# Hevagog/as-cops-and-thieves

Measured on AMD Instinct MI355X. Metric: env-steps/sec (whole node) at 4096 parallel envs, 2v1 agents, 64-ray sensors, higher is better.
Workload: dtype f64; 1 GPU; 2 cops vs 1 thieves, labyrinth map (30 hull walls / 119 planes), 4096 envs per GPU, 64 rays/agent, dt=1/60, max_step_count=400, Philox random actions, auto-reset; envs_per_gpu=4096, rays=64, agents=3, map=labyrinth, parallelism=env-sharded x1, no data-path collective, episodes_reset_per_gpu=32768, burn_in_steps=600

## Files before the change

as_cops_and_thieves_amd/csrc/cat_sim_fan.h:

```cpp
constexpr int kFeatNear = 63;
constexpr int kItemCap = 128;
constexpr int kPassJ = 8;
constexpr int kFanBytes = 2 * kItemCap * 8 + kItemCap * 2 + kPassJ * kLanes * 2;
constexpr int kGroupRays = 256;

__device__ __forceinline__ void poly_query_feat(const Lds &L, float cmax, bool wall, int sh, double r, double cx, double cy, double ax, double ay,
                                                double bx, double by, double r2, double &alpha, int &feat)
{
    const int fc = wall ? L.fc[sh] : 0, first = fc & 0xFFFF, count = fc >> 16;
    const double rsum = r + r2, rr = rsum * rsum;
    const float axf = (float)ax, ayf = (float)ay;
    const float dxf = (float)(bx - ax), dyf = (float)(by - ay);
    const float len2 = dxf * dxf + dyf * dyf, len = sqrtf(len2);
    const float e1 = 1e-6f * (fabsf(axf) + fabsf(ayf) + cmax + 512.0f);
    const float thr = ((float)rsum + 0.01f) * len * 1.00001f + 0.25f + 64.0f * e1;
    const float s_lo = -((float)rsum + 1.0f) * len, s_hi = len2 + ((float)rsum + 1.0f) * len;
    const bool bevels = rsum > 0.0;
    unsigned pm = 0u, vm = wall ? 0u : 1u;
    const double *pl0 = L.planes + 8 * first;
    {
        typedef float f32x2 __attribute__((ext_vector_type(2)));
        const float *q = L.p32 + kPairF * (wall ? L.fp[sh] : 0);
        const f32x2 ax2 = {axf, axf}, ay2 = {ayf, ayf}, dx2 = {dxf, dxf}, dy2 = {dyf, dyf};
        const f32x2 len3 = {3.0f * len, 3.0f * len}, four = {4.0f, 4.0f};
// ... 815 lines not shown
                    L.itm[t] = (unsigned short)(lane | (id << 6) | ((i - i0) << 12));
                    L.itbb[t] = tbb;
                }
                L.itemidx[(jj - jj0) * kLanes + lane] = (unsigned short)t;
                n_items += c;
            }
            const int jj1 = jj;
            wave_sync();
            PHASE(pc, 5);
            for (int t0 = 0; t0 < n_items; t0 += kLanes) {
                const int t = t0 + lane;
                if (t < n_items) {
                    const int d = L.itm[t];
                    const int il = d & 63, id = (d >> 6) & 63, ia = i0 + (d >> 12);
                    const int g2 = L.alist[r0 + il];
                    const int k2 = ((g2 >> 6) - (ia - i0) * cpa) * kLanes + (g2 & 63);
                    const double2 o2 = *reinterpret_cast<const double2 *>(L.fpos + 2 * ia);
                    const double cbx = o2.x + L.rayd[2 * k2], cby = o2.y + L.rayd[2 * k2 + 1];
                    double alpha = 2.0;
                    int feat = 0;
                    {
                        const bool wall = id < S;
                        const int j = wall ? 0 : id - S;
                        const bool inside = wall ? (id == L.anear[2 * ia] || id == L.anear[2 * ia + 1]) : ((((unsigned)L.adn[ia] >> j) & 1u) != 0u);
                        if (inside) { alpha = 0.0; feat = kFeatNear; }
                        else {
                            int f;
                            poly_query_feat(L, cmax, wall, wall ? id : 0, wall ? wall_r : rc, L.ftc[2 * j], L.ftc[2 * j + 1], o2.x, o2.y, cbx, cby, r2, alpha, f);
                            feat = f < 0 ? 0 : f;
                        }
                    }
                    L.ialpha[t] = alpha; L.itm[t] = (unsigned short)((id << 6) | feat);
                }
            }
            wave_sync();
            PHASE(pc, 6);
            for (int q = jj0; q < jj1; q++) {
                const int t = cnt > q ? (int)L.itemidx[(q - jj0) * kLanes + lane] : 0xFFFF;
                if (t != 0xFFFF) {
                    const double al = L.ialpha[t];
                    if (al < best_a && L.itbb[t] < best_a) { best_a = al; best_fi = L.itm[t]; }
                }
            }
            wave_sync();
            PHASE(pc, 7);
            jj0 = jj1;
        }
        unsigned d16 = d_empty, ty = CAT_EMPTY;
        int best = -1;
        if (best_fi >= 0) {
            const double bx = ax + L.rayd[2 * k], by = ay + L.rayd[2 * k + 1];
            best = best_fi >> 6;
            const int f = best_fi & 63;
            const double t = best_a;
            double px = bx, py = by;
            if (f != kFeatNear) {
                const bool wall = best < S;
                const int fc = wall ? L.fc[best] : 0, first = fc & 0xFFFF, count = fc >> 16;
                if (wall && f < count) {
                    const double2 n = *reinterpret_cast<const double2 *>(L.planes + 8 * (first + f));
                    px = (ax * (1.0 - t) + bx * t) - n.x * r2;
                    py = (ay * (1.0 - t) + by * t) - n.y * r2;
                } else {
                    double2 v = *reinterpret_cast<const double2 *>(L.planes + 8 * (first + (wall ? f - count : 0)) + 2);
                    if (!wall) { v.x = L.ftc[2 * (best - S)]; v.y = L.ftc[2 * (best - S) + 1]; }
                    circle_hit_point(v.x, v.y, ax, ay, bx, by, t, r2, px, py);
                }
            }
            d16 = obs_distance_f16(px, py, ax, ay);
            ty = (best < S) ? CAT_WALL : ((best - S) >= n_cops ? CAT_THIEF : CAT_COP);
        }
        if (on) {
            const int q = i * R + k;
            L.od[q] = (unsigned short)d16;
            L.ot[q] = (unsigned char)ty;
            if (la.out.hit_shape) la.out.hit_shape[(size_t)env * A * R + q] = best;
            const unsigned want = i < n_cops ? CAT_THIEF : CAT_COP;
            if (rew_mode && ty == want) __hip_atomic_fetch_min(&L.dmin[i], d16, __ATOMIC_RELAXED, __HIP_MEMORY_SCOPE_WORKGROUP);
        }
        PHASE(pc, 8);
    }
}

template <class D>
__device__ void rewards_and_positions(const Lds &L, const Params &p, const LaunchArgs &la, int lane, int rew_mode,
                                      int captured, int timeout, GAS const float *cop_lut, GAS const float *thief_lut, LateOut &late)
{
    const int A = D::A(p);
    late.reward = 0.0f; late.tp16 = 0;
    if (rew_mode && lane < A && la.out.reward) {
        const unsigned my_dmin = L.dmin[lane];
        const bool is_cop = lane < D::n_cops(p);
        float r;
        if (captured) r = is_cop ? 1.0f : -1.0f;
        else if (timeout) r = is_cop ? -1.0f : 1.0f;
        else if (my_dmin < 0x10000u) r = (is_cop ? cop_lut : thief_lut)[my_dmin & 0x7FFFu];
        else r = is_cop ? (float)(-0.02 - 0.02) : (float)0.15;
        late.reward = r;
    }
    if (lane < 2 * A) late.tp16 = f64_to_f16(L.fpos[lane]);
}
__device__ __forceinline__ void await_reward(LateOut &late) { asm volatile("" : "+v"(late.reward)); }

__device__ __forceinline__ void wide_store(void *gdst, const void *lsrc, int n, int lane)
{
    const unsigned long long ga = (unsigned long long)gdst;
    if (((ga | (unsigned)n) & 15u) == 0) {
        for (int o = lane; o < n / 16; o += kLanes) ((GAS u32x4 *)gdst)[o] = reinterpret_cast<const u32x4 *>(lsrc)[o];
    } else if (((ga | (unsigned)n) & 3u) == 0) {
        for (int o = lane; o < n / 4; o += kLanes) ((GAS unsigned *)gdst)[o] = reinterpret_cast<const unsigned *>(lsrc)[o];
    } else if (((ga | (unsigned)n) & 1u) == 0) {
        for (int o = lane; o < n / 2; o += kLanes) ((GAS unsigned short *)gdst)[o] = reinterpret_cast<const unsigned short *>(lsrc)[o];
    } else {
        for (int o = lane; o < n; o += kLanes) ((GAS unsigned char *)gdst)[o] = reinterpret_cast<const unsigned char *>(lsrc)[o];
    }
}

template <class D>
__device__ __forceinline__ void stage_shared_observations(const Lds &L, const Params &p, int lane)
{
    const int A = D::A(p), R = D::R(p);
    for (int k = lane; k < R; k += kLanes) {
        for (int team = 0; team < 2; team++) {
            const int lo = team ? D::n_cops(p) : 0, hi = team ? A : D::n_cops(p);
            unsigned ty = CAT_EMPTY, d = 0;
            for (int i = lo; i < hi; i++)
                if (ty == CAT_EMPTY) { ty = L.ot[i * R + k]; d = L.od[i * R + k]; }
            L.st[team * R + k] = (unsigned char)ty;
            L.sd[team * R + k] = (unsigned short)d;
        }
    }
    wave_sync();
}

template <class D>
__device__ __forceinline__ void emit_observations(const Lds &L, const Params &p, const LaunchArgs &la, long long env, int lane,
                                                  int rew_mode, const LateOut &late)
{
    const int A = D::A(p), R = D::R(p);
    if (rew_mode && lane < A && la.out.reward) la.out.reward[(size_t)env * A + lane] = late.reward;
    if (lane < 2 * A && la.out.team_positions) la.out.team_positions[(size_t)env * A * 2 + lane] = (unsigned short)late.tp16;
    const size_t g0 = (size_t)env * A * R;
    if (la.out.obs_distance) wide_store(la.out.obs_distance + g0, L.od, A * R * 2, lane);
    if (la.out.obs_type) wide_store(la.out.obs_type + g0, L.ot, A * R, lane);
    if (la.out.shared_distance) wide_store(la.out.shared_distance + (size_t)env * 2 * R, L.sd, 2 * R * 2, lane);
    if (la.out.shared_type) wide_store(la.out.shared_type + (size_t)env * 2 * R, L.st, 2 * R, lane);
}

template <class D>
__device__ int termination_captured(const Lds &L, const Params &p, int S, int lane)
{
    const int A = D::A(p), nc = D::n_cops(p), npairs = (A - nc) * nc;
    bool within = false;
    if (lane < npairs) {
        const int t = nc + lane / nc, c = lane % nc;
        const double ddx = L.pos[2 * t] - L.pos[2 * c], ddy = L.pos[2 * t + 1] - L.pos[2 * c + 1];
        within = sqrt(ddx * ddx + ddy * ddy) < p.term_radius;
    }
    unsigned long long cand = __ballot(within);
    while (cand) {
        {
            const int pair = __builtin_ctzll(cand);
            cand &= cand - 1;
            const int t = nc + pair / nc, c = pair % nc;
            const double ax = L.pos[2 * t], ay = L.pos[2 * t + 1], bx = L.pos[2 * c], by = L.pos[2 * c + 1];
            const double dx = bx - ax, dy = by - ay, idx = 1.0 / dx, idy = 1.0 / dy;
            bool any = false;
            for (int base = 0; base < S; base += kLanes) {
                const int s = base + lane;
                bool hit = false;
                if (s < S) {
                    bool visit = true;
                    if (p.gate && !(D::kTree && S == 1)) visit = bb_segment_query(L.bb + kBB * s, ax, ay, dx, dy, idx, idy) < 1.0;
                    if (visit) {
                        SegInfo info = {0, 1.0, bx, by};
                        if (poly_point_distance(L, s, p.wall_r, ax, ay) <= 0.0) { info.hit = 1; info.alpha = 0.0; }
                        else poly_segment_query(L, s, p.wall_r, ax, ay, bx, by, 0.0, info);
                        hit = info.hit && info.alpha < 1.0;
                    }
                }
                any = any || (__ballot(hit) != 0ull);
            }
            if (!any) return 1;
// ... 5 lines not shown
```

as_cops_and_thieves_amd/csrc/cat_sim_scheduler.h:

```cpp
template <class D>
__device__ __forceinline__ Lds carve(const Params &p, char *smem, const MapDesc &md, int slot, int wave)
{
    Lds L;
    const int S = md.S, P = md.P, W = p.wpb;
    L.bb = reinterpret_cast<const double *>(smem);
    L.planes = L.bb + kBB * S;
    L.p32 = reinterpret_cast<const float *>(L.planes + 8 * P);
    L.fc = reinterpret_cast<const int *>(L.planes + geo_rest_doubles(md));
    L.fp = L.fc + S;
    L.rayd = reinterpret_cast<const double *>(smem + p.lds_map_bytes - 16 * D::R(p));
    L.ctrl = reinterpret_cast<int *>(smem + p.lds_map_bytes);
    char *w = smem + p.lds_map_bytes + ctrl_bytes(W) + slot * p.lds_env_bytes;
    const int A = D::A(p), R = D::R(p), NPs = D::NP(p) > 0 ? D::NP(p) : 1;
    L.rec = w;
    double *d = reinterpret_cast<double *>(w);
    L.pos = d; d += 2 * A; L.vel = d; d += 2 * A; L.vb = d; d += 2 * A; L.tc = d; d += 2 * A;
    L.leaf = d; d += 4 * A;
    L.cnt = reinterpret_cast<int *>(d);
    d = reinterpret_cast<double *>(w + D::hot_bytes(p));
    L.wjn = d; d += A * kK; L.pjn = d; d += NPs;
    {
        int *ri = reinterpret_cast<int *>(d);
        L.wsh = ri; ri += A * kK; L.wag = ri; ri += A * kK; L.pag = ri;
    }
// ... 67 lines not shown
        dm.S = m.S; dm.P = m.P; dm.A = m.A; dm.n_regions = m.n_regions; dm.f64_off = m.f64_off; dm.i32_off = m.i32_off; dm.cmax = m.cmax; dm.PP = m.PP;
        dg.x0 = g.x0; dg.y0 = g.y0; dg.inv_cell = g.inv_cell; dg.nx = g.nx; dg.ny = g.ny; dg.off_base = g.off_base; dg.ent_base = g.ent_base;
        dg.coff_base = g.coff_base; dg.cent_base = g.cent_base; dg.crow_base = g.crow_base; dg.span = g.span; dg.row_base = g.row_base; dg.span_tick = g.span_tick;
    }
    __syncthreads();
}

template <class D>
__device__ __forceinline__ void load_cold(const Lds &L, const Params &p, int env, int lane)
{
    const int A = D::A(p), NPs = D::NP(p) > 0 ? D::NP(p) : 1;
    const int hot16 = D::hot_bytes(p) / 16, cold16 = (D::rec_bytes(p) - D::hot_bytes(p)) / 16;
    u32x4 *dst = reinterpret_cast<u32x4 *>(L.rec) + hot16;
    if (uni(L.cnt[3]) != 0) {
        GAS const u32x4 *src = (GAS const u32x4 *)(G(p.state) + (size_t)env * D::rec_bytes(p)) + hot16;
        for (int o = lane; o < cold16; o += kLanes) dst[o] = src[o];
    } else {
        const int nd2 = 2 * (A * kK + NPs);
        for (int o = lane; o < cold16; o += kLanes) {
            u32x4 v;
#pragma unroll
            for (int q = 0; q < 4; q++) {
                const int j = 4 * o + q - nd2;
                v[q] = (j >= 0 && (j < A * kK || (j >= 2 * A * kK && j < 2 * A * kK + NPs))) ? 0xFFFFFFFFu : 0u;
            }
            dst[o] = v;
        }
    }
    wave_sync();
}

template <class D>
__device__ __forceinline__ void load_state(const Lds &L, const Params &p, int env, int lane)
{
    GAS const u32x4 *src = (GAS const u32x4 *)(G(p.state) + (size_t)env * D::rec_bytes(p));
    u32x4 *dst = reinterpret_cast<u32x4 *>(L.rec);
    for (int o = lane; o < D::hot_bytes(p) / 16; o += kLanes) dst[o] = src[o];
    wave_sync();
    load_cold<D>(L, p, env, lane);
}

struct StateRegs { u32x4 v; };
template <class D>
__device__ __forceinline__ void fetch_state(StateRegs &r, const Params &p, int env, int lane)
{
    GAS const u32x4 *src = (GAS const u32x4 *)(G(p.state) + (size_t)(env < 0 ? 0 : env) * D::rec_bytes(p));
    if (lane < D::hot_bytes(p) / 16) r.v = src[lane];
}
template <class D>
__device__ __forceinline__ void commit_state(const Lds &L, const StateRegs &r, const Params &p, int lane)
{
    u32x4 *dst = reinterpret_cast<u32x4 *>(L.rec);
    if (lane < D::hot_bytes(p) / 16) dst[lane] = r.v;
    wave_sync();
}

template <class D>
__device__ __forceinline__ void store_state(const Lds &L, const Params &p, int env, int lane)
{
    wave_sync();
    const int A = D::A(p);
    const bool mine = (lane < A * kK && L.wsh[lane] >= 0) || (lane < D::NP(p) && L.pag[lane] >= 0);
    const bool live = __ballot(mine) != 0ull;
    if (lane == 0) L.cnt[3] = live ? 1 : 0;
    wave_sync();
    GAS u32x4 *dst = (GAS u32x4 *)(G(p.state) + (size_t)env * D::rec_bytes(p));
    const u32x4 *src = reinterpret_cast<const u32x4 *>(L.rec);
    const int n16 = (live ? D::rec_bytes(p) : D::hot_bytes(p)) / 16;
    for (int o = lane; o < n16; o += kLanes) dst[o] = src[o];
}

#ifdef CAT_WAVE_SPREAD
__device__ unsigned long long g_wave_t[8 * 65536];
__device__ unsigned long long g_slot_t[16 * 65536];
extern "C" int cat_debug_spread(unsigned long long *out, int n)
{
    return hipMemcpyFromSymbol(out, HIP_SYMBOL(g_wave_t), sizeof(unsigned long long) * 8 * n) == hipSuccess ? 0 : -1;
}
extern "C" int cat_debug_slot_times(unsigned long long *out, int n)
{
    return hipMemcpyFromSymbol(out, HIP_SYMBOL(g_slot_t), sizeof(unsigned long long) * 16 * n) == hipSuccess ? 0 : -1;
}
#define SSPREAD(slot_, i) do { if (kOneTick && lane0 == 0 && (i) < 14) g_slot_t[16 * (blockIdx.x * (blockDim.x / kLanes) + (slot_)) + (i)] = __builtin_amdgcn_s_memrealtime(); } while (0)
#define WSPREAD(i) do { if (kOneTick && lane0 == 0) g_wave_t[8 * (blockIdx.x * (blockDim.x / kLanes) + wave) + (i)] = ((i) < 4 || (i) > 5) ? __builtin_amdgcn_s_memrealtime() : __builtin_readcyclecounter(); } while (0)
#else
#define WSPREAD(i) do {} while (0)
#define SSPREAD(slot_, i) do {} while (0)
#endif
__device__ __forceinline__ int ctrl_add(int *w, int lane)
{
    int v = 0;
    if (lane == 0) v = __hip_atomic_fetch_add(w, 1, __ATOMIC_RELAXED, __HIP_MEMORY_SCOPE_WORKGROUP);
    return uni(v);
}
__device__ __forceinline__ void copy_snapshot(const Lds &L, int A, int lane)
{
    if (lane < 8 * A) L.spawn[lane] = L.pos[lane + (lane < 2 * A ? 0 : 4 * A)];
    wave_sync();
}

__device__ __forceinline__ void publish_slot(const Lds &L, int wave, int lane, int n_units)
{
    __builtin_amdgcn_fence(__ATOMIC_RELEASE, "workgroup");
    if (lane == 0) __hip_atomic_store(&L.ctrl[4 * wave + 2], n_units, __ATOMIC_RELAXED, __HIP_MEMORY_SCOPE_WORKGROUP);
}

template <class D>
__device__ __forceinline__ void slot_writeback(const Lds &Ls, const Params &p, const LaunchArgs &la, int e_s, long long env_out, int lane,
                                               int tick, bool store_rec, int step2, int captured2, int timeout2, int rcount,
                                               GAS const float *cop_lut, GAS const float *thief_lut, PhaseClock &pc)
{
    LateOut late;
    rewards_and_positions<D>(Ls, p, la, lane, tick, captured2, timeout2, cop_lut, thief_lut, late);
    stage_shared_observations<D>(Ls, p, lane);
    await_reward(late);
    PHASE(pc, 17);
    const unsigned char term = (unsigned char)(captured2 || timeout2);
    if (lane == 0) {
        Ls.cnt[0] = step2; Ls.cnt[2] = rcount >= 0 ? 0 : term;
        if (rcount >= 0) Ls.cnt[1] = rcount;
    }
    if (store_rec) store_state<D>(Ls, p, e_s, lane);
    PHASE(pc, 18);
    emit_observations<D>(Ls, p, la, env_out, lane, tick, late);
    PHASE(pc, 19);
    if (tick && lane == 0) {
        if (la.out.terminated) la.out.terminated[env_out] = term;
        if (la.out.truncated) la.out.truncated[env_out] = (unsigned char)timeout2;
        if (la.out.winner) la.out.winner[env_out] = (signed char)(captured2 ? 0 : (timeout2 ? 1 : -1));
    }
}

__device__ __forceinline__ int opaque_v(int v) { asm volatile("" : "+v"(v)); __builtin_assume((unsigned)v < (unsigned)kLanes); return v; }
typedef const LaunchArgs __attribute__((address_space(4))) *LaunchArgsK;
typedef const Params __attribute__((address_space(4))) *ParamsK;
__device__ __forceinline__ LaunchArgsK kernarg_launch_args()
{
    return (LaunchArgsK)((const char __attribute__((address_space(4))) *)__builtin_amdgcn_kernarg_segment_ptr() + 8);
}
__device__ __forceinline__ const BlockDesc *block_desc_lds(char *smem, const Params &p, int W)
{
    return reinterpret_cast<const BlockDesc *>(smem + p.lds_map_bytes + 16 * W);
}
typedef const Prologue __attribute__((address_space(4))) *PrologueK;
__device__ __forceinline__ PrologueK kernarg_prologue()
{
    return (PrologueK)((const char __attribute__((address_space(4))) *)__builtin_amdgcn_kernarg_segment_ptr() + 8 + sizeof(LaunchArgs));
}
__device__ __forceinline__ Params prologue_params(PrologueK pk, int &uniform)
{
    Params q;
    q.lds_map_bytes = pk->lds_map_bytes; q.lds_env_bytes = pk->lds_env_bytes; q.lds_union_bytes = pk->lds_union_bytes; q.wpb = pk->wpb;
    q.A = pk->A; q.R = pk->R; q.NP = pk->NP; q.maxc = pk->maxc; q.n_cops = pk->n_cops; q.rec_bytes = pk->rec_bytes; q.hot_bytes = pk->hot_bytes;
    q.N = pk->N; uniform = pk->uniform; q.lds_pool_off = pk->lds_pool_off; q.pool_mask = pk->pool_mask; q.grp_rays = pk->grp_rays;
    q.work_env = pk->work_env; q.block_desc = pk->block_desc; q.state = pk->state;
    q.geo_f64 = pk->geo_f64; q.geo_i32 = pk->geo_i32; q.ray_dx = pk->ray_dx; q.ray_dy = pk->ray_dy;
    q.cop_lut = pk->cop_lut; q.thief_lut = pk->thief_lut;
    asm volatile("" : "+s"(q.lds_map_bytes), "+s"(q.lds_env_bytes), "+s"(q.lds_union_bytes), "+s"(q.wpb), "+s"(q.A), "+s"(q.R), "+s"(q.NP),
                      "+s"(q.n_cops), "+s"(q.rec_bytes), "+s"(q.hot_bytes), "+s"(q.N), "+s"(uniform), "+s"(q.lds_pool_off), "+s"(q.pool_mask), "+s"(q.grp_rays), "+s"(q.work_env), "+s"(q.block_desc), "+s"(q.state),
                      "+s"(q.geo_f64), "+s"(q.geo_i32), "+s"(q.ray_dx), "+s"(q.ray_dy), "+s"(q.cop_lut), "+s"(q.thief_lut));
    return q;
}
__device__ __forceinline__ void copy_desc(BlockDesc &d, const BlockDesc &s)
{
    d.md.S = s.md.S; d.md.P = s.md.P; d.md.A = s.md.A; d.md.n_regions = s.md.n_regions; d.md.f64_off = s.md.f64_off; d.md.i32_off = s.md.i32_off;
    d.md.cmax = s.md.cmax; d.md.PP = s.md.PP;
    d.gd.x0 = s.gd.x0; d.gd.y0 = s.gd.y0; d.gd.inv_cell = s.gd.inv_cell; d.gd.nx = s.gd.nx; d.gd.ny = s.gd.ny; d.gd.off_base = s.gd.off_base;
    d.gd.ent_base = s.gd.ent_base; d.gd.coff_base = s.gd.coff_base; d.gd.cent_base = s.gd.cent_base; d.gd.crow_base = s.gd.crow_base; d.gd.span = s.gd.span;
    d.gd.row_base = s.gd.row_base; d.gd.span_tick = s.gd.span_tick;
}
__device__ __forceinline__ void prologue_env_desc(const Params &q, int uniform, int W, int wave, int &env, BlockDesc &bd0)
{
    copy_desc(bd0, *(const BlockDesc *)(const void *)&kernarg_prologue()->bd);
    const int e = blockIdx.x * W + wave;
    env = e < q.N ? e : -1;
    if (!uniform) {
        env = uni(q.work_env[e]);
        copy_desc(bd0, q.block_desc[blockIdx.x]);
    }
}

template <class D>
__device__ __forceinline__ void run_units(const Params *pp0, LaunchArgsK lap0, char *smem, int W, int wave, int lane0, int tick, PhaseClock &pc)
{
    unsigned fin_mask = 0u;
    bool own_first = true;
    int *const ctrl0 = reinterpret_cast<int *>(smem + launder((ParamsK)pp0)->lds_map_bytes);
    GAS const float *cop_lut = launder(G(launder((ParamsK)pp0)->cop_lut)), *thief_lut = launder(G(launder((ParamsK)pp0)->thief_lut));
    for (;;) {
        int slot, e_s, last_unit;
        {
            const int lane = opaque_v(lane0);
            int *const ctrl = ctrl0;
            int e_l = -1, nu_l = 0, cl_l = 0;
            if (lane < W) {
                e_l = ctrl[4 * lane + 3];
                nu_l = __hip_atomic_load(&ctrl[4 * lane + 2], __ATOMIC_RELAXED, __HIP_MEMORY_SCOPE_WORKGROUP);
                cl_l = __hip_atomic_load(&ctrl[4 * lane + 0], __ATOMIC_RELAXED, __HIP_MEMORY_SCOPE_WORKGROUP);
            }
            const unsigned open = (unsigned)__ballot(e_l >= 0 && nu_l > 0 && cl_l < nu_l);
            const unsigned unpublished = (unsigned)__ballot(e_l >= 0 && nu_l == 0);
            if (open == 0u) {
                if (unpublished == 0u) break;
                __builtin_amdgcn_s_sleep(8);
                continue;
            }
            if (own_first && ((open >> wave) & 1u)) slot = wave;
            else {
                const unsigned rot = wave == 0 ? open : ((open >> wave) | (open << (32 - wave)));
                slot = (wave + __builtin_ctz(rot)) & 31;
            }
            own_first = false;
            slot = uni(slot);
// ... 255 lines not shown
            } else {
                PHASE(pc, 9);
#ifndef CAT_ABL_NOPHYS
                physics_env<D>(Ls, p, uni(K->md.S), lane, pc);
#endif
                PHASE(pc, 10);
            }
            lds_release();
            SSPREAD(slot, 3 + 2 * unit);
            int d = 0;
            if (lane == 0) d = __hip_atomic_fetch_add(&ctrl[4 * slot + 1], 1, __ATOMIC_RELAXED, __HIP_MEMORY_SCOPE_WORKGROUP);
            fin = uni(d) == n_units - 1;
            PHASE(pc, 23);
        }
        if (!fin) continue;
        {
            const int lane = opaque_v(lane0);
            const Params &p = *(const Params *)launder((ParamsK)pp0);
            const LaunchArgs &la = *(const LaunchArgs *)launder(lap0);
            int *const ctrl = reinterpret_cast<int *>(smem + p.lds_map_bytes);
            const BlockDesc *const K = block_desc_lds(smem, p, W);
            lds_acquire();
            PHASE(pc, 16);
            SSPREAD(slot, 12);
            const int e_s = uni(ctrl[4 * slot + 3]);
            const Lds Ls = carve<D>(p, smem, K->md, slot, wave);
            const long long eo = (long long)t * p.N + e_s;
            const int step2 = uni(Ls.flags[0]), captured2 = uni(Ls.flags[1]), timeout2 = uni(Ls.flags[2]), rcount = uni(Ls.flags[3]);
            const bool last = t + 1 >= T;
#ifndef CAT_ABL_NOWB
            slot_writeback<D>(Ls, p, la, e_s, eo, lane, 1, last, step2, captured2, timeout2, rcount, lut_c, lut_t, pc);
#else
            (void)eo; (void)step2; (void)captured2; (void)timeout2; (void)rcount; (void)la;
#endif
            wave_sync();
            SSPREAD(slot, 13);
            if (!last) { pend = slot; pend_t = t + 1; }
            else if (lane == 0) __hip_atomic_store((unsigned *)&ctrl[4 * slot], kRwFinished, __ATOMIC_RELAXED, __HIP_MEMORY_SCOPE_WORKGROUP);
        }
    }
    PHASE(pc, 11);
    WSPREAD(3); WSPREAD(5);
    pc.flush(lane0);
}

template <class D>
__global__ __launch_bounds__(kMaxWaves *kLanes) void rollout_kernel(const Params *__restrict__ pp0, const LaunchArgs la0, const Prologue)
{
    rollout_body<D, false>(pp0, la0);
}

template <class D>
__global__ __launch_bounds__(kMaxWaves *kLanes) void step_kernel(const Params *__restrict__ pp0, const LaunchArgs la0, const Prologue)
{
    rollout_body<D, true>(pp0, la0);
}

#ifdef CAT_WB_COUNTS
__device__ unsigned long long g_wb_counts[8];
extern "C" int cat_debug_wb_counts(unsigned long long *out8, int reset)
{
    unsigned long long h[8];
    if (hipMemcpyFromSymbol(h, HIP_SYMBOL(g_wb_counts), sizeof h) != hipSuccess) return -1;
    for (int i = 0; i < 8; i++) out8[i] = h[i];
    if (reset) { memset(h, 0, sizeof h); if (hipMemcpyToSymbol(HIP_SYMBOL(g_wb_counts), h, sizeof h) != hipSuccess) return -1; }
    return 0;
}
#endif
template <class T> __device__ __forceinline__ T *slot_ptr(T *p0, int sl, int envb) { return (T *)((char *)const_cast<typename std::remove_const<T>::type *>(p0) + sl * envb); }
constexpr unsigned kPoolValid = 0x80000000u;
constexpr double kPoolEmptyRows = 0.05;
#ifndef CAT_POOL_ROUND
#define CAT_POOL_ROUND 60
#endif
#ifndef CAT_POOL_MIN_PARTIAL
#define CAT_POOL_MIN_PARTIAL 40
#endif
#ifndef CAT_POOL_PATIENCE
#define CAT_POOL_PATIENCE 3
#endif
constexpr int kPoolRound = CAT_POOL_ROUND;
constexpr int kPoolMinPartial = CAT_POOL_MIN_PARTIAL;
constexpr int kPoolPatience = CAT_POOL_PATIENCE;
#ifdef CAT_FAULT_INJECT
constexpr int kSpinLimit = 1 << 14;
#else
constexpr int kSpinLimit = 1 << 22;
#endif
__device__ __forceinline__ int *pool_ctl(char *smem, const Params &p, int W) { return reinterpret_cast<int *>(smem + p.lds_map_bytes + 16 * W + kWgConstBytes - 8); }
static_assert(sizeof(BlockDesc) <= kWgConstBytes - 8, "the pool counters live behind the BlockDesc");

template <bool kExact>
__device__ __forceinline__ int ring_pos(const Params &p, unsigned i)
{
    if constexpr (!kExact) return (int)(i & (unsigned)p.pool_mask);
    const unsigned t = __umulhi(p.pool_magic, i);
    const unsigned q = (t + ((i - t) >> 1)) >> p.pool_shift;
    return (int)(i - q * (unsigned)(p.pool_mask + 1));
}

template <class D, bool kExact>
__device__ __forceinline__ int pool_sort(const Lds &L, const Params &p, const LaunchArgs &la, const GridDesc &gd, long long env, int slot, int lane,
                                         int *pctl, unsigned long long *pool)
{
    const int A = D::A(p), R = D::R(p);
    const unsigned d_empty = f64_to_f16(p.ray_length);
    const unsigned long long lt_mask = (1ull << lane) - 1ull;
    const int cpa = (R + kLanes - 1) / kLanes, nch = A * cpa;
    const int my_cell = lane < A ? L.acell[lane] : -1;
    const int my_dk0 = lane < A * A ? L.dk0[lane] : 0, my_dcnt = lane < A * A ? L.dcnt[lane] : 0;
    int n_res = 0;
    for (int c0 = 0; c0 < nch; c0 += 4) {
        unsigned wrow[4] = {0u, 0u, 0u, 0u};
#pragma unroll
        for (int q = 0; q < 4; q++) {
            if (c0 + q < nch) {
                const int i = (c0 + q) / cpa, k = ((c0 + q) - i * cpa) * kLanes + lane;
                const int cell = __builtin_amdgcn_readlane(my_cell, i);
                const size_t r = (cell < 0 || k >= R) ? 0 : (size_t)cell * R + k;
                wrow[q] = ((GAS const unsigned *)G(p.grid_rows))[gd.row_base + r];
            }
        }
#pragma unroll
        for (int q = 0; q < 4; q++) {
            if (c0 + q < nch) {
                const int i = (c0 + q) / cpa, k = ((c0 + q) - i * cpa) * kLanes + lane;
                const int cell = __builtin_amdgcn_readlane(my_cell, i);
                const bool in = k < R;
                const unsigned rowv = (in && cell >= 0) ? wrow[q] : 0u;
                unsigned dynmask = 0;
                if (in)
                    for (int j = 0; j < A; j++) {
                        if (j == i) continue;
                        const int dc = __builtin_amdgcn_readlane(my_dcnt, i * A + j) & 0xFFFF, dk = __builtin_amdgcn_readlane(my_dk0, i * A + j);
                        int rel = k - dk; if (rel < 0) rel += R;
                        if (rel < dc) dynmask |= 1u << j;
                    }
                bool act = rowv != 0u || dynmask != 0u;
                const unsigned long long m = __ballot(act);
                const int n = __popcll(m);
                int base = 0;
                if (n) {
                    if (lane == 0) base = __hip_atomic_fetch_add(&pctl[1], n, __ATOMIC_RELAXED, __HIP_MEMORY_SCOPE_WORKGROUP);
                    base = uni(base);
                }
                unsigned long long *const e = &pool[act ? ring_pos<kExact>(p, (unsigned)(base + __popcll(m & lt_mask))) : 0];
#ifdef CAT_FAULT_INJECT
                if (slot == 0 && c0 + q == 0 && n && lane == (int)__builtin_ctzll(m)) act = false;
#endif
                for (int spins = 0; __ballot(act && __hip_atomic_load(e, __ATOMIC_RELAXED, __HIP_MEMORY_SCOPE_WORKGROUP) != 0ull) != 0ull;)
                    if (++spins >= kSpinLimit) { if (lane == 0) atomicOr(p.err_word, CAT_DEVERR_SCHEDULER); break; }
                if (act) {
                    const unsigned meta = kPoolValid | ((unsigned)slot << 24) | ((unsigned)i << 16) | (dynmask << 8) | (unsigned)k;
                    __hip_atomic_store(e, ((unsigned long long)meta << 32) | rowv, __ATOMIC_RELAXED, __HIP_MEMORY_SCOPE_WORKGROUP);
                } else if (in && (rowv == 0u && dynmask == 0u)) {
                    const int o = i * R + k;
                    L.od[o] = (unsigned short)d_empty;
                    L.ot[o] = (unsigned char)CAT_EMPTY;
                    if (la.out.hit_shape) la.out.hit_shape[(size_t)env * A * R + o] = -1;
                }
                n_res += __popcll(__ballot(in && (rowv == 0u && dynmask == 0u)));
            }
        }
    }
    return n_res;
}
// ... 165 lines not shown

template <class D, bool kOneTick, bool kExact>
__device__ __forceinline__ void rollout_body_pool(const Params *__restrict__ pp0, const LaunchArgs &la0)
{
    extern __shared__ __align__(16) char smem[];
    const int lane0 = threadIdx.x % kLanes;
    const int wave = uni(threadIdx.x / kLanes);
    const LaunchArgsK lap0 = kernarg_launch_args();
    PhaseClock pc;
    WSPREAD(0); WSPREAD(4);
    int env, T, W;
    GAS const float *lut_c, *lut_t;
    {
        int uniform;
        const Params q = prologue_params(kernarg_prologue(), uniform);
        const Params &p = *(const Params *)(ParamsK)pp0;
        lut_c = G(q.cop_lut); lut_t = G(q.thief_lut);
        const int lane = lane0;
        W = uni((int)(blockDim.x / kLanes));
        T = kOneTick ? 1 : la0.T;
        WSPREAD(6);
        int *const ctrl = reinterpret_cast<int *>(smem + q.lds_map_bytes);
        BlockDesc bd0;
        prologue_env_desc(q, uniform, W, wave, env, bd0);
        const MapDesc &md0 = bd0.md;
#ifdef CAT_WAVE_SPREAD
        { int e_ = env, s_ = md0.S; asm volatile("" : "+s"(e_), "+v"(s_)); WSPREAD(7); }
#endif
        if (lane < 4) ctrl[4 * wave + lane] = lane == 3 ? env : ((lane == 0 && env < 0) ? (int)kRwFinished : 0);
        {
            u32x4 *pz = reinterpret_cast<u32x4 *>(smem + q.lds_pool_off);
            const u32x4 z = {0u, 0u, 0u, 0u};
            for (int o = threadIdx.x; o < (q.pool_mask + 1) / 2; o += blockDim.x) pz[o] = z;
            if (threadIdx.x == 0) { int *pc2 = pool_ctl(smem, q, W); pc2[0] = 0; pc2[1] = 0; }
        }
        StateRegs sregs;
        fetch_state<D>(sregs, q, env, lane);
        stage_map<D>(q, smem, md0, &bd0, const_cast<BlockDesc *>(block_desc_lds(smem, q, W)));
        PHASE(pc, 0);
        WSPREAD(1);
        if (env >= 0) {
            const Lds L = carve<D>(q, smem, md0, wave, wave);
            commit_state<D>(L, sregs, q, lane);
            load_cold<D>(L, p, env, lane);
            PHASE(pc, 1);
        }
    }
    unsigned todo = env >= 0 ? 1u << wave : 0u;
    unsigned wbm = 0u;
    int hint = wave, idle = 0;
    int stall = 0, moved_sig = 0;
    unsigned w_seen = 0u;
    for (;;) {
        while (todo) {
            const int lane = opaque_v(lane0);
            const Params &p = *(const Params *)launder((ParamsK)pp0);
            const LaunchArgs &la = *(const LaunchArgs *)launder(lap0);
            int *const ctrl = reinterpret_cast<int *>(smem + p.lds_map_bytes);
            const BlockDesc *const K = block_desc_lds(smem, p, W);
            const int slot = uni(__builtin_ctz(todo));
            todo &= todo - 1;
            SSPREAD(slot, 0);
            const int e_s = uni(ctrl[4 * slot + 3]), t = uni(ctrl[4 * slot + 2]);
            const Lds Ls = carve<D>(p, smem, K->md, slot, wave);
            int ap = 0;
            if (la.actions && lane < D::A(p)) ap = la.actions[((size_t)t * p.N + e_s) * D::A(p) + lane];
            if (lane == 0) ctrl[4 * slot + 1] = 0;
            const int n2 = slot_front<D>(Ls, (ParamsK)pp0, la, K->md, K->gd, e_s, lane, ap, la.synth_tick + (unsigned long long)t, 0, pc);
            lds_release();
            if (lane == 0) __hip_atomic_store((unsigned *)&ctrl[4 * slot], rw_make(t + 1, n2), __ATOMIC_RELAXED, __HIP_MEMORY_SCOPE_WORKGROUP);
            PHASE(pc, 3);
            const int n_res = pool_sort<D, kExact>(Ls, p, la, K->gd, (long long)t * p.N + e_s, slot, lane, pool_ctl(smem, p, W), reinterpret_cast<unsigned long long *>(smem + p.lds_pool_off));
            lds_release();
            const int add = n_res + (n2 == 0 ? 1 : 0);
            int old = 0;
            if (lane == 0) old = __hip_atomic_fetch_add(&ctrl[4 * slot + 1], add, __ATOMIC_RELAXED, __HIP_MEMORY_SCOPE_WORKGROUP);
            if (add > 0 && uni(old) + add == D::A(p) * D::R(p) + 1) wbm |= 1u << slot;
            hint = slot;
            WSPREAD(2); SSPREAD(slot, 1);
        }
#ifdef CAT_WB_COUNTS
        if (wbm && lane0 == 0) { const int k_ = __popc(wbm); atomicAdd(&g_wb_counts[k_ > 7 ? 7 : k_], 1ull); }
#endif
        while (wbm) {
            const int lane = opaque_v(lane0);
            const Params &p = *(const Params *)launder((ParamsK)pp0);
            const LaunchArgs &la = *(const LaunchArgs *)launder(lap0);
            int *const ctrl = reinterpret_cast<int *>(smem + p.lds_map_bytes);
            const BlockDesc *const K = block_desc_lds(smem, p, W);
            const int slot = uni(__builtin_ctz(wbm));
            wbm &= wbm - 1;
            lds_acquire();
            PHASE(pc, 16);
            SSPREAD(slot, 12);
            const int e_s = uni(ctrl[4 * slot + 3]), t = uni(ctrl[4 * slot + 2]);
            const Lds Ls = carve<D>(p, smem, K->md, slot, wave);
            const long long eo = (long long)t * p.N + e_s;
            const int step2 = uni(Ls.flags[0]), captured2 = uni(Ls.flags[1]), timeout2 = uni(Ls.flags[2]), rcount = uni(Ls.flags[3]);
            const bool last = t + 1 >= T;
            slot_writeback<D>(Ls, p, la, e_s, eo, lane, 1, last, step2, captured2, timeout2, rcount, lut_c, lut_t, pc);
            wave_sync();
            SSPREAD(slot, 13);
            if (!last) { if (lane == 0) ctrl[4 * slot + 2] = t + 1; todo |= 1u << slot; }
            else if (lane == 0) __hip_atomic_store((unsigned *)&ctrl[4 * slot], kRwFinished, __ATOMIC_RELAXED, __HIP_MEMORY_SCOPE_WORKGROUP);
        }
        if (todo) continue;
        int base, n, slot = -1;
        {
            const int lane = opaque_v(lane0);
            const Params &p = *(const Params *)launder((ParamsK)pp0);
            int *const ctrl = reinterpret_cast<int *>(smem + p.lds_map_bytes);
            int *const pctl = pool_ctl(smem, p, W);
            unsigned w_l = kRwFinished;
            if (lane < W) w_l = __hip_atomic_load((unsigned *)&ctrl[4 * lane], __ATOMIC_RELAXED, __HIP_MEMORY_SCOPE_WORKGROUP);
            int hd = 0, tl = 0;
            if (lane == 0) { hd = __hip_atomic_load(&pctl[0], __ATOMIC_RELAXED, __HIP_MEMORY_SCOPE_WORKGROUP); tl = __hip_atomic_load(&pctl[1], __ATOMIC_RELAXED, __HIP_MEMORY_SCOPE_WORKGROUP); }
            hd = uni(hd); tl = uni(tl);
            const int avail = tl - hd;
            const unsigned open = (unsigned)__ballot(rw_next(w_l) < rw_units(w_l));
            if (avail >= kPoolRound || (open == 0u && (avail >= kPoolMinPartial || (avail > 0 && idle >= kPoolPatience)))) {
                base = hd; n = avail < kPoolRound ? avail : kPoolRound;
                int seen = hd;
                if (lane == 0) __hip_atomic_compare_exchange_strong(&pctl[0], &seen, hd + n, __ATOMIC_RELAXED, __ATOMIC_RELAXED, __HIP_MEMORY_SCOPE_WORKGROUP);
                if (uni(seen) != hd) continue;
            } else if (open != 0u) {
                n = 0; base = 0;
                unsigned key = 0xFFFFFFFFu;
                if (rw_next(w_l) < rw_units(w_l)) key = ((unsigned)rw_epoch(w_l) << 5) | (unsigned)((lane - hint) & 31);
#define CAT_ROW_MIN(SH) { const unsigned o_ = (unsigned)__builtin_amdgcn_update_dpp((int)key, (int)key, 0x120 + SH, 0xF, 0xF, false); key = o_ < key ? o_ : key; }
                CAT_ROW_MIN(8) CAT_ROW_MIN(4) CAT_ROW_MIN(2) CAT_ROW_MIN(1)
#undef CAT_ROW_MIN
                slot = uni((hint + (int)(key & 31u)) & 31);
                const unsigned wv = (unsigned)__builtin_amdgcn_readlane((int)w_l, slot);
                unsigned seen = wv;
                if (lane == 0)
                    __hip_atomic_compare_exchange_strong((unsigned *)&ctrl[4 * slot], &seen, wv + 1u, __ATOMIC_RELAXED, __ATOMIC_RELAXED, __HIP_MEMORY_SCOPE_WORKGROUP);
                if ((unsigned)uni((int)seen) != wv) continue;
                hint = slot;
            } else {
                if (avail == 0 && __ballot(kOneTick ? (w_l == 0u) : (w_l != kRwFinished)) == 0ull) break;
                ++idle;
                {
                    const bool moved = __ballot(w_l != w_seen) != 0ull || hd + tl != moved_sig;
                    w_seen = w_l; moved_sig = hd + tl;
                    stall = moved ? 0 : stall + 1;
                }
                if (stall > kSpinLimit) { if (lane == 0) atomicOr(p.err_word, CAT_DEVERR_SCHEDULER); break; }
                __builtin_amdgcn_s_sleep(4);
                PHASE(pc, 21);
                continue;
            }
            idle = 0;
            lds_acquire();
            PHASE(pc, 22);
        }
        {
            const int lane = opaque_v(lane0);
            const Params &p = *(const Params *)launder((ParamsK)pp0);
            const LaunchArgs &la = *(const LaunchArgs *)launder(lap0);
            int *const ctrl = reinterpret_cast<int *>(smem + p.lds_map_bytes);
            const BlockDesc *const K = block_desc_lds(smem, p, W);
            if (n > 0) {
                const Lds L0 = carve<D>(p, smem, K->md, 0, wave);
                wbm |= pool_round<D, kExact>(L0, p, la, uni(K->md.S), K->md.cmax, base, n, lane, ctrl, reinterpret_cast<unsigned long long *>(smem + p.lds_pool_off), pc);
            } else {
                const Lds Ls = carve<D>(p, smem, K->md, slot, wave);
                SSPREAD(slot, 2);
                PHASE(pc, 9);
                physics_env<D>(Ls, p, uni(K->md.S), lane, pc);
                PHASE(pc, 10);
                lds_release();
                SSPREAD(slot, 3);
                int old = 0;
                if (lane == 0) old = __hip_atomic_fetch_add(&ctrl[4 * slot + 1], 1, __ATOMIC_RELAXED, __HIP_MEMORY_SCOPE_WORKGROUP);
                if (uni(old) + 1 == D::A(p) * D::R(p) + 1) wbm |= 1u << slot;
            }
            PHASE(pc, 23);
        }
    }
    PHASE(pc, 11);
    WSPREAD(3); WSPREAD(5);
    pc.flush(lane0);
}

template <class D, bool kExact = false>
__global__ __launch_bounds__(kMaxWaves *kLanes) void rollout_kernel_pooled(const Params *__restrict__ pp0, const LaunchArgs la0, const Prologue)
{
// ... 164 lines not shown
```

Before: 135.0 million env-steps/s.

## Batch slot writebacks to overlap reward LUT loads across multiple slots

The writeback loop now takes up to four ready slots at once. It first issues the reward lookup-table global loads for all of them, then stages shared observations for all of them, and only then waits for the rewards and finishes each slot's writeback. Before, each slot paid its own global-load latency in series, and this change is meant to hide that latency across slots. In exchange it holds more registers for the reward array, adds more carve and LDS passes, and delays the publishing of the first slot's completion until the whole batch is staged.

```diff
diff --git a/as_cops_and_thieves_amd/csrc/cat_sim_fan.h b/as_cops_and_thieves_amd/csrc/cat_sim_fan.h
--- a/as_cops_and_thieves_amd/csrc/cat_sim_fan.h
+++ b/as_cops_and_thieves_amd/csrc/cat_sim_fan.h
@@ -921,23 +921,35 @@
     }
 }
 
+struct RewardReq { GAS const float *src; float r; };
+template <class D>
+__device__ __forceinline__ RewardReq reward_request(const Lds &L, const Params &p, const LaunchArgs &la, int lane, int rew_mode,
+                                                    int captured, int timeout, GAS const float *cop_lut, GAS const float *thief_lut)
+{
+    RewardReq q = {nullptr, 0.0f};
+    if (rew_mode && lane < D::A(p) && la.out.reward) {
+        const unsigned my_dmin = L.dmin[lane];
+        const bool is_cop = lane < D::n_cops(p);
+        if (captured) q.r = is_cop ? 1.0f : -1.0f;
+        else if (timeout) q.r = is_cop ? -1.0f : 1.0f;
+        else if (my_dmin < 0x10000u) q.src = (is_cop ? cop_lut : thief_lut) + (my_dmin & 0x7FFFu);
+        else q.r = is_cop ? (float)(-0.02 - 0.02) : (float)0.15;
+    }
+    return q;
+}
+template <class D>
+__device__ __forceinline__ unsigned team_positions_f16(const Lds &L, const Params &p, int lane)
+{
+    return lane < 2 * D::A(p) ? f64_to_f16(L.fpos[lane]) : 0u;
+}
 template <class D>
 __device__ void rewards_and_positions(const Lds &L, const Params &p, const LaunchArgs &la, int lane, int rew_mode,
                                       int captured, int timeout, GAS const float *cop_lut, GAS const float *thief_lut, LateOut &late)
 {
-    const int A = D::A(p);
-    late.reward = 0.0f; late.tp16 = 0;
-    if (rew_mode && lane < A && la.out.reward) {
-        const unsigned my_dmin = L.dmin[lane];
-        const bool is_cop = lane < D::n_cops(p);
-        float r;
-        if (captured) r = is_cop ? 1.0f : -1.0f;
-        else if (timeout) r = is_cop ? -1.0f : 1.0f;
-        else if (my_dmin < 0x10000u) r = (is_cop ? cop_lut : thief_lut)[my_dmin & 0x7FFFu];
-        else r = is_cop ? (float)(-0.02 - 0.02) : (float)0.15;
-        late.reward = r;
-    }
-    if (lane < 2 * A) late.tp16 = f64_to_f16(L.fpos[lane]);
+    const RewardReq q = reward_request<D>(L, p, la, lane, rew_mode, captured, timeout, cop_lut, thief_lut);
+    late.reward = q.r;
+    if (q.src) late.reward = *q.src;
+    late.tp16 = team_positions_f16<D>(L, p, lane);
 }
 __device__ __forceinline__ void await_reward(LateOut &late) { asm volatile("" : "+v"(late.reward)); }
 
diff --git a/as_cops_and_thieves_amd/csrc/cat_sim_scheduler.h b/as_cops_and_thieves_amd/csrc/cat_sim_scheduler.h
--- a/as_cops_and_thieves_amd/csrc/cat_sim_scheduler.h
+++ b/as_cops_and_thieves_amd/csrc/cat_sim_scheduler.h
@@ -173,10 +173,12 @@
     return hipMemcpyFromSymbol(out, HIP_SYMBOL(g_slot_t), sizeof(unsigned long long) * 16 * n) == hipSuccess ? 0 : -1;
 }
 #define SSPREAD(slot_, i) do { if (kOneTick && lane0 == 0 && (i) < 14) g_slot_t[16 * (blockIdx.x * (blockDim.x / kLanes) + (slot_)) + (i)] = __builtin_amdgcn_s_memrealtime(); } while (0)
+#define SSPREAD_V(slot_, i, v_) do { if (kOneTick && lane0 == 0) g_slot_t[16 * (blockIdx.x * (blockDim.x / kLanes) + (slot_)) + (i)] = (v_); } while (0)
 #define WSPREAD(i) do { if (kOneTick && lane0 == 0) g_wave_t[8 * (blockIdx.x * (blockDim.x / kLanes) + wave) + (i)] = ((i) < 4 || (i) > 5) ? __builtin_amdgcn_s_memrealtime() : __builtin_readcyclecounter(); } while (0)
 #else
 #define WSPREAD(i) do {} while (0)
 #define SSPREAD(slot_, i) do {} while (0)
+#define SSPREAD_V(slot_, i, v_) do {} while (0)
 #endif
 __device__ __forceinline__ int ctrl_add(int *w, int lane)
 {
@@ -197,15 +199,10 @@
 }
 
 template <class D>
-__device__ __forceinline__ void slot_writeback(const Lds &Ls, const Params &p, const LaunchArgs &la, int e_s, long long env_out, int lane,
-                                               int tick, bool store_rec, int step2, int captured2, int timeout2, int rcount,
-                                               GAS const float *cop_lut, GAS const float *thief_lut, PhaseClock &pc)
-{
-    LateOut late;
-    rewards_and_positions<D>(Ls, p, la, lane, tick, captured2, timeout2, cop_lut, thief_lut, late);
-    stage_shared_observations<D>(Ls, p, lane);
-    await_reward(late);
-    PHASE(pc, 17);
+__device__ __forceinline__ void slot_writeback_finish(const Lds &Ls, const Params &p, const LaunchArgs &la, int e_s, long long env_out, int lane,
+                                                      int tick, bool store_rec, int step2, int captured2, int timeout2, int rcount,
+                                                      const LateOut &late, PhaseClock &pc)
+{
     const unsigned char term = (unsigned char)(captured2 || timeout2);
     if (lane == 0) {
         Ls.cnt[0] = step2; Ls.cnt[2] = rcount >= 0 ? 0 : term;
@@ -220,6 +217,19 @@
         if (la.out.truncated) la.out.truncated[env_out] = (unsigned char)timeout2;
         if (la.out.winner) la.out.winner[env_out] = (signed char)(captured2 ? 0 : (timeout2 ? 1 : -1));
     }
+}
+
+template <class D>
+__device__ __forceinline__ void slot_writeback(const Lds &Ls, const Params &p, const LaunchArgs &la, int e_s, long long env_out, int lane,
+                                               int tick, bool store_rec, int step2, int captured2, int timeout2, int rcount,
+                                               GAS const float *cop_lut, GAS const float *thief_lut, PhaseClock &pc)
+{
+    LateOut late;
+    rewards_and_positions<D>(Ls, p, la, lane, tick, captured2, timeout2, cop_lut, thief_lut, late);
+    stage_shared_observations<D>(Ls, p, lane);
+    await_reward(late);
+    PHASE(pc, 17);
+    slot_writeback_finish<D>(Ls, p, la, e_s, env_out, lane, tick, store_rec, step2, captured2, timeout2, rcount, late, pc);
 }
 
 __device__ __forceinline__ int opaque_v(int v) { asm volatile("" : "+v"(v)); __builtin_assume((unsigned)v < (unsigned)kLanes); return v; }
@@ -641,6 +651,10 @@
 constexpr int kPoolRound = CAT_POOL_ROUND;
 constexpr int kPoolMinPartial = CAT_POOL_MIN_PARTIAL;
 constexpr int kPoolPatience = CAT_POOL_PATIENCE;
+#ifndef CAT_WB_BATCH
+#define CAT_WB_BATCH 4
+#endif
+constexpr int kWbBatch = CAT_WB_BATCH;
 #ifdef CAT_FAULT_INJECT
 constexpr int kSpinLimit = 1 << 14;
 #else
@@ -972,27 +986,71 @@
 #ifdef CAT_WB_COUNTS
         if (wbm && lane0 == 0) { const int k_ = __popc(wbm); atomicAdd(&g_wb_counts[k_ > 7 ? 7 : k_], 1ull); }
 #endif
+#ifdef CAT_WAVE_SPREAD
+        {
+            int q_ = 0;
+            for (unsigned m_ = wbm; m_; m_ &= m_ - 1, q_++) {
+                const int s_ = __builtin_ctz(m_);
+                SSPREAD_V(s_, 14, __builtin_amdgcn_s_memrealtime());
+                SSPREAD_V(s_, 15, (unsigned long long)((q_ << 8) | __popc(wbm)));
+            }
+        }
+#endif
         while (wbm) {
-            const int lane = opaque_v(lane0);
-            const Params &p = *(const Params *)launder((ParamsK)pp0);
-            const LaunchArgs &la = *(const LaunchArgs *)launder(lap0);
-            int *const ctrl = reinterpret_cast<int *>(smem + p.lds_map_bytes);
-            const BlockDesc *const K = block_desc_lds(smem, p, W);
-            const int slot = uni(__builtin_ctz(wbm));
-            wbm &= wbm - 1;
             lds_acquire();
             PHASE(pc, 16);
-            SSPREAD(slot, 12);
-            const int e_s = uni(ctrl[4 * slot + 3]), t = uni(ctrl[4 * slot + 2]);
-            const Lds Ls = carve<D>(p, smem, K->md, slot, wave);
-            const long long eo = (long long)t * p.N + e_s;
-            const int step2 = uni(Ls.flags[0]), captured2 = uni(Ls.flags[1]), timeout2 = uni(Ls.flags[2]), rcount = uni(Ls.flags[3]);
-            const bool last = t + 1 >= T;
-            slot_writeback<D>(Ls, p, la, e_s, eo, lane, 1, last, step2, captured2, timeout2, rcount, lut_c, lut_t, pc);
-            wave_sync();
-            SSPREAD(slot, 13);
-            if (!last) { if (lane == 0) ctrl[4 * slot + 2] = t + 1; todo |= 1u << slot; }
-            else if (lane == 0) __hip_atomic_store((unsigned *)&ctrl[4 * slot], kRwFinished, __ATOMIC_RELAXED, __HIP_MEMORY_SCOPE_WORKGROUP);
+            unsigned batch = wbm;
+            for (int q = 0; q < kWbBatch && wbm; q++) wbm &= wbm - 1;
+            batch &= ~wbm;
+            float rew[kWbBatch];
+#pragma unroll
+            for (int q = 0; q < kWbBatch; q++) rew[q] = 0.0f;
+            int j = 0;
+            for (unsigned m = batch; m; m &= m - 1, j++) {
+                const int lane = opaque_v(lane0);
+                const Params &p = *(const Params *)launder((ParamsK)pp0);
+                const LaunchArgs &la = *(const LaunchArgs *)launder(lap0);
+                const BlockDesc *const K = block_desc_lds(smem, p, W);
+                const int slot = uni(__builtin_ctz(m));
+                SSPREAD(slot, 12);
+                const Lds Ls = carve<D>(p, smem, K->md, slot, wave);
+                const RewardReq rq = reward_request<D>(Ls, p, la, lane, 1, uni(Ls.flags[1]), uni(Ls.flags[2]), lut_c, lut_t);
+#pragma unroll
+                for (int q = 0; q < kWbBatch; q++)
+                    if (j == q) { rew[q] = rq.r; if (rq.src) rew[q] = *rq.src; }
+            }
+            for (unsigned m = batch; m; m &= m - 1) {
+                const Params &p = *(const Params *)launder((ParamsK)pp0);
+                stage_shared_observations<D>(carve<D>(p, smem, block_desc_lds(smem, p, W)->md, uni(__builtin_ctz(m)), wave), p, opaque_v(lane0));
+            }
+#pragma unroll
+            for (int q = 0; q < kWbBatch; q++) asm volatile("" : "+v"(rew[q]));
+            PHASE(pc, 17);
+            j = 0;
+            for (unsigned m = batch; m; m &= m - 1, j++) {
+                const int lane = opaque_v(lane0);
+                const Params &p = *(const Params *)launder((ParamsK)pp0);
+                const LaunchArgs &la = *(const LaunchArgs *)launder(lap0);
+                const BlockDesc *const K = block_desc_lds(smem, p, W);
+                int *const ctrl = reinterpret_cast<int *>(smem + p.lds_map_bytes);
+                const int slot = uni(__builtin_ctz(m));
+                const Lds Ls = carve<D>(p, smem, K->md, slot, wave);
+                LateOut lt;
+                lt.reward = rew[0];
+#pragma unroll
+                for (int q = 1; q < kWbBatch; q++)
+                    if (j == q) lt.reward = rew[q];
+                lt.tp16 = team_positions_f16<D>(Ls, p, lane);
+                const int e_s = uni(ctrl[4 * slot + 3]), t = uni(ctrl[4 * slot + 2]);
+                const long long eo = (long long)t * p.N + e_s;
+                const int step2 = uni(Ls.flags[0]), captured2 = uni(Ls.flags[1]), timeout2 = uni(Ls.flags[2]), rcount = uni(Ls.flags[3]);
+                const bool last = t + 1 >= T;
+                slot_writeback_finish<D>(Ls, p, la, e_s, eo, lane, 1, last, step2, captured2, timeout2, rcount, lt, pc);
+                wave_sync();
+                SSPREAD(slot, 13);
+                if (!last) { if (lane == 0) ctrl[4 * slot + 2] = t + 1; todo |= 1u << slot; }
+                else if (lane == 0) __hip_atomic_store((unsigned *)&ctrl[4 * slot], kRwFinished, __ATOMIC_RELAXED, __HIP_MEMORY_SCOPE_WORKGROUP);
+            }
         }
         if (todo) continue;
         int base, n, slot = -1;
```

Measured after the change: 133.2 million env-steps/s. 1.4% lower.
